# risc0/zeth

Measured on AMD Instinct MI355X. Metric: segments/sec, higher is better.
Workload: dtype u32

## Files before the change

zeth_amd/csrc/common.h:

```cpp
#pragma once
#include <hip/hip_runtime.h>

#include <atomic>
#include <cstdarg>
#include <cstdio>
#include <cstdlib>
#include <cstring>
#include <map>
#include <string>
#include <vector>

#include "../../include/zkhal.h"
#include "fp.h"
#include "noise.h"

namespace zkh {

inline const char* make_err(const char* fmt, ...) {
    char buf[512];
    va_list ap;
    va_start(ap, fmt);
    vsnprintf(buf, sizeof buf, fmt, ap);
    va_end(ap);
    return strdup(buf);
// ... 7 lines not shown
    do {                                 \
        const char* _err = (expr);       \
        if (_err) return _err;           \
    } while (0)
#define ZKH_REQUIRE(cond, ...)                         \
    do {                                               \
        if (!(cond)) return zkh::make_err(__VA_ARGS__); \
    } while (0)

constexpr int ZKH_P2_PTAB = 414;
constexpr int TW_BITS = 12;
constexpr int TW_SIZE = 1 << TW_BITS;
constexpr int TW_HI_BITS = 14;
constexpr int TW_HI_SIZE = 1 << TW_HI_BITS;
constexpr int MAX_LOG_N = TW_BITS + TW_HI_BITS;
constexpr int LDS_TW_LOG = 12;

struct DeviceTables {
    uint32_t* rc;
    uint32_t* diag;
    uint32_t* tw_fwd_lo; uint32_t* tw_fwd_hi;
    uint32_t* tw_rev_lo; uint32_t* tw_rev_hi;
    uint32_t* tile_fwd;  uint32_t* tile_rev;
    uint32_t* layer_fwd; uint32_t* layer_rev;
    uint32_t* layer_fwd_lazy;
    uint32_t* shift_lo;  uint32_t* shift_hi;
};

struct ProfAgg { uint64_t calls = 0; double ms = 0; double bytes = 0; };
struct ProfPending { std::string name; hipEvent_t a, b; double bytes; };

}

struct zkh_alloc_t {
    void* ptr;
    size_t bytes;
    std::atomic<int> refs;
    bool owned;
    zkh_ctx* ctx;
    zkh_alloc_t(void* p, size_t b, int r, bool o, zkh_ctx* c) : ptr(p), bytes(b), refs(r), owned(o), ctx(c) {}
};

struct zkh_buf {
    zkh_alloc_t* a;
    size_t off, len;
    std::atomic<int> refs;
    zkh_buf(zkh_alloc_t* al, size_t o, size_t l, int r) : a(al), off(o), len(l), refs(r) {}
    uint32_t* ptr() const { return (uint32_t*)a->ptr + off; }
// ... 68 lines not shown
```

zeth_amd/csrc/fp.h:

```cpp
#pragma once
#include <stdint.h>

#if defined(__HIPCC__)
#include <hip/hip_runtime.h>
#define ZKH_HD __host__ __device__ __forceinline__
#else
#define ZKH_HD inline
#endif

namespace zkh {

constexpr uint32_t P = 2013265921u;
constexpr uint32_t PINV = 0x88000001u;
constexpr uint32_t NEG_PINV = 0x77ffffffu;
constexpr uint32_t R1 = 268435454u;
constexpr uint32_t R2 = 1172168163u;
constexpr uint32_t INVALID = 0xffffffffu;

struct Fp {
    uint32_t v;
    ZKH_HD Fp() : v(0) {}
    ZKH_HD explicit constexpr Fp(uint32_t raw, int) : v(raw) {}
    static ZKH_HD Fp raw(uint32_t r) { return Fp(r, 0); }
    static ZKH_HD Fp one() { return Fp(R1, 0); }
// ... 33 lines not shown
    return d;
#else
    return (int64_t)((uint64_t)acc + (uint64_t)((int64_t)a * b));
#endif
}
ZKH_HD int64_t mad_i64_k(int32_t a, int32_t b_uniform, int64_t acc) {
#if defined(__HIP_DEVICE_COMPILE__)
    int64_t d; uint64_t carry;
    asm("v_mad_i64_i32 %0, %1, %2, %3, %4" : "=v"(d), "=s"(carry) : "v"(a), "s"(b_uniform), "v"(acc));
    return d;
#else
    return (int64_t)((uint64_t)acc + (uint64_t)((int64_t)a * b_uniform));
#endif
}
ZKH_HD int64_t mul_i64(int32_t a, int32_t b) {
#if defined(__HIP_DEVICE_COMPILE__)
    int64_t d; uint64_t carry;
    asm("v_mad_i64_i32 %0, %1, %2, %3, 0" : "=v"(d), "=s"(carry) : "v"(a), "v"(b));
    return d;
#else
    return (int64_t)a * b;
#endif
}
ZKH_HD int32_t smont_reduce(int64_t t) {
    const int32_t m = (int32_t)((uint32_t)t * NEG_PINV);
    return (int32_t)(mad_i64_k(m, (int32_t)P, t) >> 32);
}
ZKH_HD int32_t smont(int32_t a, int32_t b) {
    const int64_t t = (int64_t)a * b;
    const int32_t m = (int32_t)((uint32_t)t * NEG_PINV);
    const int64_t s = t + (int64_t)m * (int64_t)P;
    return (int32_t)(s >> 32);
}
ZKH_HD uint32_t canon(int32_t x) { const uint32_t u = (uint32_t)x, v = u + P; return v < u ? v : u; }
ZKH_HD int32_t center(uint32_t x) { return (int32_t)(x - (x > (P - 1) / 2 ? P : 0u)); }
ZKH_HD uint32_t mul_mod(uint32_t a, uint32_t b) { return mont_reduce((uint64_t)a * b); }

ZKH_HD Fp operator+(Fp a, Fp b) { return Fp::raw(add_mod(a.v, b.v)); }
ZKH_HD Fp operator-(Fp a, Fp b) { return Fp::raw(sub_mod(a.v, b.v)); }
ZKH_HD Fp operator*(Fp a, Fp b) { return Fp::raw(mul_mod(a.v, b.v)); }
ZKH_HD Fp operator-(Fp a) { return Fp::raw(a.v ? P - a.v : 0); }
ZKH_HD bool operator==(Fp a, Fp b) { return a.v == b.v; }
ZKH_HD Fp& operator+=(Fp& a, Fp b) { a = a + b; return a; }
ZKH_HD Fp& operator-=(Fp& a, Fp b) { a = a - b; return a; }
ZKH_HD Fp& operator*=(Fp& a, Fp b) { a = a * b; return a; }

ZKH_HD Fp fp_encode(uint32_t x) { return Fp::raw(mul_mod(R2, x % P)); }
ZKH_HD uint32_t fp_decode(Fp a) { return mul_mod(1u, a.v); }
ZKH_HD Fp fp_pow(Fp a, uint64_t e) {
    Fp r = Fp::one();
    while (e) { if (e & 1) r = r * a; a = a * a; e >>= 1; }
    return r;
}
ZKH_HD Fp fp_inv(Fp a) { return fp_pow(a, P - 2); }

constexpr uint32_t NBETA_CANON = P - 11;
// ... 79 lines not shown
```

zeth_amd/csrc/hal.hip:

```cpp
#include <algorithm>

#include "common.h"

#include <sys/random.h>
#include "poseidon2.h"
#include "ntt_lazy.h"
#include "../../include/zkh_poseidon2_consts.h"

using namespace zkh;

extern "C" void zkh_free_error(const char* e) { free((void*)e); }
#if ZKH_P2_CONSTS_ARE_PLACEHOLDER
extern "C" const char* zkh_version(void) { return "zkhal-mi355x 0.2.0 (gfx950; poseidon2_consts=placeholder)"; }
#elif ZKH_P2_CONSTS_ARE_DERIVED
extern "C" const char* zkh_version(void) { return "zkhal-mi355x 0.2.0 (gfx950; poseidon2_consts=derived)"; }
#else
extern "C" const char* zkh_version(void) { return "zkhal-mi355x 0.2.0 (gfx950; poseidon2_consts=upstream)"; }
#endif

namespace zkh {

const char* pool_alloc(zkh_ctx* c, size_t bytes, void** out) {
    bytes = (bytes + 255) & ~(size_t)255;
    if (bytes == 0) bytes = 256;
// ... 132 lines not shown
        delete c;
        return make_err("hipStreamCreateWithFlags: %s", hipGetErrorString(se));
    }
    if (const char* err = ctx_init_tables(c)) {
        zkh_ctx_destroy(c);
        return err;
    }
    *out = c;
    return nullptr;
}
static const char* ctx_init_tables(zkh_ctx* c) {
    Fp g = fp_encode(137);
    for (int k = 0; k <= 27; k++) {
        Fp w = fp_pow(g, 1ull << (27 - k));
        c->rou_fwd[k] = w.v;
        c->rou_rev[k] = fp_inv(w).v;
    }
    Fp wf = Fp::raw(c->rou_fwd[MAX_LOG_N]), wr = Fp::raw(c->rou_rev[MAX_LOG_N]);
    ZKH_TRY(upload(&c->tab.tw_fwd_lo, powers(wf, TW_SIZE)));
    ZKH_TRY(upload(&c->tab.tw_fwd_hi, powers(fp_pow(wf, TW_SIZE), TW_HI_SIZE)));
    ZKH_TRY(upload(&c->tab.tw_rev_lo, powers(wr, TW_SIZE)));
    ZKH_TRY(upload(&c->tab.tw_rev_hi, powers(fp_pow(wr, TW_SIZE), TW_HI_SIZE)));
    ZKH_TRY(upload(&c->tab.tile_fwd, powers(Fp::raw(c->rou_fwd[LDS_TW_LOG]), 1 << (LDS_TW_LOG - 1))));
    ZKH_TRY(upload(&c->tab.tile_rev, powers(Fp::raw(c->rou_rev[LDS_TW_LOG]), 1 << (LDS_TW_LOG - 1))));
    {
        std::vector<uint32_t> lf(1 << LDS_TW_LOG, R1), lr(1 << LDS_TW_LOG, R1);
        for (int j = 1; j <= LDS_TW_LOG; j++) {
            auto pf = powers(Fp::raw(c->rou_fwd[j]), (size_t)1 << (j - 1)), pr = powers(Fp::raw(c->rou_rev[j]), (size_t)1 << (j - 1));
            for (size_t e = 0; e < pf.size(); e++) { lf[((size_t)1 << (j - 1)) + e] = pf[e]; lr[((size_t)1 << (j - 1)) + e] = pr[e]; }
        }
        ZKH_TRY(upload(&c->tab.layer_fwd, lf));
        ZKH_TRY(upload(&c->tab.layer_rev, lr));
        static_assert(LAZY_TAB_LOG == LDS_TW_LOG, "the lazy table covers the per-layer tables");
        std::vector<uint32_t> lz(LAZY_TAB_WORDS);
        lazy_layer_table(lz.data(), lf.data());
        ZKH_TRY(upload(&c->tab.layer_fwd_lazy, lz));
    }
    Fp three = fp_encode(3);
    ZKH_TRY(upload(&c->tab.shift_lo, powers(three, TW_SIZE)));
    ZKH_TRY(upload(&c->tab.shift_hi, powers(fp_pow(three, TW_SIZE), TW_HI_SIZE)));
    ZKH_TRY(upload(&c->tab.rc, std::vector<uint32_t>(24 * 29)));
    ZKH_TRY(upload(&c->tab.diag, std::vector<uint32_t>(ZKH_P2_PTAB)));
    ZKH_TRY(zkh_poseidon2_set_constants(c, ZKH_P2_ROUND_CONSTANTS, ZKH_P2_M_INT_DIAG));
    ZKH_TRY(ntt_device_init(c));
    ZKH_HIP(hipMalloc((void**)&c->d_fail, 8));
    ZKH_HIP(hipMemsetAsync(c->d_fail, 0, 8, c->stream));
    ZKH_HIP(hipHostMalloc((void**)&c->h_fail, 8, hipHostMallocDefault));
    c->h_fail[0] = c->h_fail[1] = 0;
    return nullptr;
}
extern "C" const char* zkh_ctx_trim(zkh_ctx* c) {
    bind_thread(c);
    ZKH_HIP(hipStreamSynchronize(c->stream));
    for (auto& kv : c->pool) (void)hipFree(kv.second);
    c->pool.clear(); c->pool_bytes = 0;
    return nullptr;
}
extern "C" void zkh_ctx_memory(const zkh_ctx* c, size_t* live, size_t* cached, size_t* peak) {
    if (live) *live = c->live_bytes;
    if (cached) *cached = c->pool_bytes;
    if (peak) *peak = c->peak_bytes;
}
extern "C" void zkh_ctx_destroy(zkh_ctx* c) {
    if (!c) return;
    (void)hipSetDevice(c->device);
    (void)hipStreamSynchronize(c->stream);
    for (auto& kv : c->pool) (void)hipFree(kv.second);
    uint32_t* t[] = {c->tab.rc, c->tab.diag, c->tab.tw_fwd_lo, c->tab.tw_fwd_hi, c->tab.tw_rev_lo, c->tab.tw_rev_hi,
                     c->tab.tile_fwd, c->tab.tile_rev, c->tab.shift_lo, c->tab.shift_hi, c->tab.layer_fwd, c->tab.layer_rev, c->tab.layer_fwd_lazy};
    for (auto p : t) (void)hipFree(p);
    for (auto& p : c->pending) { (void)hipEventDestroy(p.a); (void)hipEventDestroy(p.b); }
    for (auto ev : c->event_pool) (void)hipEventDestroy(ev);
    if (c->pinned) (void)hipHostFree(c->pinned);
    if (c->d_fail) (void)hipFree(c->d_fail);
    if (c->h_fail) (void)hipHostFree(c->h_fail);
    for (auto& kv : c->host_blocks) (void)hipHostFree(kv.first);
    (void)hipStreamDestroy(c->stream);
    delete c;
}
static const char* check_device_fail(zkh_ctx* c) {
    if (!c->fail_armed) return nullptr;
    c->fail_armed = false;
    const uint32_t code = c->h_fail[0], detail = c->h_fail[1];
    if (!code) return nullptr;
    (void)hipMemsetAsync(c->d_fail, 0, 8, c->stream);
    switch (code) {
    case 1: return make_err("combos_prepare_regs: register %u has size 0 or more than `cycles` words (found on the device; the call's combos are unchanged)", detail);
    case 2: return make_err("combos_prepare_regs: register %u names a combo beyond combo_count (found on the device; the call's combos are unchanged)", detail);
    case 3: return make_err("combos_prepare_regs: the register sizes add up to %u U coefficients (+ %d of the check polynomial), more than coeff_u holds (found on the device; the call's combos are unchanged)", detail, ZKH_CHECK_SIZE);
    default: return make_err("a kernel reported failure code %u (%u)", code, detail);
    }
}
// ... 373 lines not shown
```

zeth_amd/csrc/ntt.hip:

```cpp
#include "common.h"
#include "ntt_lazy.h"

using namespace zkh;

namespace {

constexpr int NTT_THREADS = 256;

struct PassParams {
    const uint32_t* in;
    uint32_t* out;
    size_t in_col_stride;
    size_t out_col_stride;
    uint32_t log_n;
    uint32_t L, R;
    uint32_t log_t;
    uint32_t expand_bits;
    uint32_t first_layer;
    uint32_t twiddle;
    uint32_t scale;
    uint32_t zk_shift;
    const uint32_t* tile_tw;
    const uint32_t* layer_tw;
    const uint32_t* tw_lo;
// ... 188 lines not shown
    __syncthreads();
    for (uint32_t e = threadIdx.x; e < H * H; e += blockDim.x) {
        const uint32_t hi2 = e >> BR_H, lo2 = e & (H - 1);
        const uint32_t shi = __brev(lo2) >> (32 - BR_H), slo = __brev(hi2) >> (32 - BR_H);
        const uint32_t src = (shi << BR_H) | slo;
        col[((size_t)hi2 << (log_n - BR_H)) | ((size_t)rmid << BR_H) | lo2] = ta[src];
        if (rmid != mid) col[((size_t)hi2 << (log_n - BR_H)) | ((size_t)mid << BR_H) | lo2] = tb[src];
    }
}
__global__ void k_bit_reverse_small(uint32_t* io, uint32_t log_n, size_t count) {
    size_t g = (size_t)blockIdx.x * blockDim.x + threadIdx.x;
    size_t n = (size_t)1 << log_n;
    if (g >= n * count) return;
    uint32_t i = (uint32_t)(g & (n - 1));
    uint32_t r = log_n ? __brev(i) >> (32 - log_n) : 0;
    if (i < r) {
        uint32_t* col = io + (g - i);
        uint32_t x = col[i], y = col[r];
        col[i] = y; col[r] = x;
    }
}


template <int LOGR, bool INVERSE, bool BASE0, int J_LO, bool LAZY = false>
__device__ __forceinline__ void radix_layers(uint32_t (&v)[1 << LOGR], const uint32_t* __restrict__ ltab,
                                             const uint32_t base_low, const int first_b) {
    constexpr int N = 1 << LOGR;
    if (!INVERSE && LAZY) {
        lazy_layers<LOGR, BASE0, J_LO>(v, ltab, base_low, first_b);
    } else if (INVERSE) {
#pragma unroll
        for (int b = LOGR - 1; b >= 0; b--) {
            const uint32_t* tw = ltab + (1u << (J_LO + b - 1));
#pragma unroll
            for (int kk = 0; kk < (1 << b); kk++) {
                const bool unit = BASE0 && kk == 0;
                const uint32_t w = unit ? 0u : tw[base_low + ((uint32_t)kk << (J_LO - 1))];
#pragma unroll
                for (int hi = 0; hi < (N >> (b + 1)); hi++) {
                    const int k = (hi << (b + 1)) | kk;
                    const uint32_t x = v[k], y = v[k + (1 << b)];
                    v[k] = add_mod(x, y);
                    v[k + (1 << b)] = unit ? sub_mod(x, y) : mul_mod(x - y + P, w);
                }
            }
        }
    } else {
#pragma unroll
        for (int b = 0; b < LOGR; b++) {
            if (b < first_b) continue;
            const uint32_t* tw = ltab + (1u << (J_LO + b - 1));
#pragma unroll
            for (int kk = 0; kk < (1 << b); kk++) {
                const bool unit = BASE0 && kk == 0;
                const uint32_t w = unit ? 0u : tw[base_low + ((uint32_t)kk << (J_LO - 1))];
#pragma unroll
                for (int hi = 0; hi < (N >> (b + 1)); hi++) {
                    const int k = (hi << (b + 1)) | kk;
                    const uint32_t x = v[k], y = unit ? v[k + (1 << b)] : mul_mod(v[k + (1 << b)], w);
                    v[k] = add_mod(x, y);
                    v[k + (1 << b)] = sub_mod(x, y);
                }
            }
        }
    }
}

template <bool INVERSE, bool LAZY = false>
__global__ __launch_bounds__(256) void k_ntt_low12(PassParams p) {
    __shared__ __attribute__((aligned(16))) uint32_t lds[4096];
    const uint32_t tid = threadIdx.x;
    const uint32_t tile = xcd_remap(blockIdx.x, p.tiles_per_col);
    const size_t base = (size_t)tile << 12;
    const uint32_t* in = p.in + (size_t)blockIdx.y * p.in_col_stride;
    uint32_t* out = p.out + (size_t)blockIdx.y * p.out_col_stride;
    const uint32_t* __restrict__ ltab = p.layer_tw;
    const uint32_t hi = tid >> 4, low = tid & 15;
    uint32_t v[16];
    if (INVERSE) {
#pragma unroll
        for (int k = 0; k < 16; k++) v[k] = in[base + k * 256 + tid];
        radix_layers<4, true, false, 9>(v, ltab, tid, 0);
#pragma unroll
        for (int k = 0; k < 16; k++) lds[k * 256 + tid] = v[k];
        __syncthreads();
#pragma unroll
        for (int k = 0; k < 16; k++) v[k] = lds[hi * 256 + k * 16 + low];
        radix_layers<4, true, false, 5>(v, ltab, low, 0);
#pragma unroll
        for (int k = 0; k < 16; k++) lds[hi * 256 + k * 16 + low] = v[k];
        __syncthreads();
#pragma unroll
        for (int q = 0; q < 4; q++) {
            const uint4 w = ((const uint4*)lds)[tid * 4 + q];
            v[4 * q] = w.x; v[4 * q + 1] = w.y; v[4 * q + 2] = w.z; v[4 * q + 3] = w.w;
        }
        radix_layers<4, true, true, 1>(v, ltab, 0, 0);
        const size_t pos0 = base + (size_t)tid * 16;
        if (p.zk_shift) {
            const uint32_t ex = __brev((uint32_t)pos0) >> (32 - p.log_n);
            const uint32_t b = mul_mod(p.sh_lo[ex & (TW_SIZE - 1)], p.sh_hi[ex >> TW_BITS]);
#pragma unroll
            for (int k = 0; k < 16; k++) v[k] = mul_mod(mul_mod(v[k], b), p.shift16[k]);
        } else if (p.scale) {
#pragma unroll
            for (int k = 0; k < 16; k++) v[k] = mul_mod(v[k], p.scale);
        }
#pragma unroll
        for (int q = 0; q < 4; q++) ((uint4*)(out + pos0))[q] = make_uint4(v[4 * q], v[4 * q + 1], v[4 * q + 2], v[4 * q + 3]);
    } else {
        const size_t pos0 = base + (size_t)tid * 16;
        if (p.expand_bits == 0) {
#pragma unroll
            for (int q = 0; q < 4; q++) {
                const uint4 w = ((const uint4*)(in + pos0))[q];
                v[4 * q] = w.x; v[4 * q + 1] = w.y; v[4 * q + 2] = w.z; v[4 * q + 3] = w.w;
            }
        } else if (p.expand_bits == 2) {
            const uint4 w = *(const uint4*)(in + (pos0 >> 2));
            v[0] = v[1] = v[2] = v[3] = w.x; v[4] = v[5] = v[6] = v[7] = w.y;
            v[8] = v[9] = v[10] = v[11] = w.z; v[12] = v[13] = v[14] = v[15] = w.w;
        } else {
#pragma unroll
            for (int k = 0; k < 16; k++) v[k] = in[(pos0 + k) >> p.expand_bits];
        }
        radix_layers<4, false, true, 1, LAZY>(v, ltab, 0, (int)p.expand_bits);
#pragma unroll
        for (int q = 0; q < 4; q++) ((uint4*)lds)[tid * 4 + q] = make_uint4(v[4 * q], v[4 * q + 1], v[4 * q + 2], v[4 * q + 3]);
        __syncthreads();
#pragma unroll
        for (int k = 0; k < 16; k++) v[k] = lds[hi * 256 + k * 16 + low];
        radix_layers<4, false, false, 5, LAZY>(v, ltab, low, 0);
#pragma unroll
        for (int k = 0; k < 16; k++) lds[hi * 256 + k * 16 + low] = v[k];
        __syncthreads();
#pragma unroll
        for (int k = 0; k < 16; k++) v[k] = lds[k * 256 + tid];
        radix_layers<4, false, false, 9, LAZY>(v, ltab, tid, 0);
#pragma unroll
        for (int k = 0; k < 16; k++) out[base + k * 256 + tid] = v[k];
    }
}

template <int RH, bool INVERSE, bool LAZY = false>
__global__ __launch_bounds__(1 << RH) void k_ntt_high(PassParams p) {
    constexpr int LT = 4;
    constexpr uint32_t TW = 1u << LT;
    extern __shared__ __attribute__((aligned(16))) uint32_t lds[];
    const uint32_t tid = threadIdx.x, t = tid & (TW - 1), g = tid >> LT;
    const uint32_t tile_id = xcd_remap(blockIdx.x, p.tiles_per_col), col = blockIdx.y;
    const uint32_t lt_bits = p.L - LT;
    const uint32_t a = tile_id >> lt_bits, lt = tile_id & ((1u << lt_bits) - 1);
    const size_t base = ((size_t)a << (p.L + RH)) + ((size_t)lt << LT);
    const uint32_t lcol = (lt << LT) + t;
    const uint32_t tw_shift = MAX_LOG_N - (p.L + RH);
    const char* in = (const char*)(p.in + (size_t)col * p.in_col_stride + base);
    char* out = (char*)(p.out + (size_t)col * p.out_col_stride + base);
    const uint32_t tb = t * 4u;
#define TILE_IN(row) (*(const uint32_t*)(in + ((((uint32_t)(row)) << (p.L + 2)) + tb)))
#define TILE_OUT(row) (*(uint32_t*)(out + ((((uint32_t)(row)) << (p.L + 2)) + tb)))
    const uint32_t* __restrict__ ltab = p.layer_tw;
    auto tmul = [](uint32_t x, uint32_t y) -> uint32_t {
        return (LAZY && !INVERSE) ? (uint32_t)smont((int32_t)x, (int32_t)y) : mul_mod(x, y);
    };
    auto root = [&](uint32_t e) -> uint32_t {
        const uint32_t ex = e << tw_shift;
        return tmul(p.tw_lo[ex & (TW_SIZE - 1)], p.tw_hi[ex >> TW_BITS]);
    };
    uint32_t tw[16];
    if (RH == 10) {
        uint32_t w0 = root(lcol * (__brev(g) >> 26));
        if (LAZY) w0 = tmul(w0, p.lazy_comp);
        const uint32_t u1 = root(lcol * 64u), v1 = root(lcol * 256u);
        const uint32_t u2 = tmul(u1, u1), u3 = tmul(u2, u1), v2 = tmul(v1, v1), v3 = tmul(v2, v1);
        const uint32_t wi[4] = {w0, tmul(w0, u2), tmul(w0, u1), tmul(w0, u3)};
#pragma unroll
        for (int i = 0; i < 4; i++) {
            tw[4 * i] = wi[i]; tw[4 * i + 1] = tmul(wi[i], v2); tw[4 * i + 2] = tmul(wi[i], v1); tw[4 * i + 3] = tmul(wi[i], v3);
        }
    } else {
        uint32_t w0 = root(lcol * (__brev(g) >> 28));
        if (LAZY) w0 = tmul(w0, p.lazy_comp);
        const uint32_t q1 = root(lcol * 16u);
        uint32_t qp[16];
        qp[0] = w0;
#pragma unroll
        for (int e = 1; e < 16; e++) qp[e] = tmul(qp[e - 1], q1);
#pragma unroll
        for (int k = 0; k < 16; k++) tw[k] = qp[__builtin_bitreverse8((unsigned char)k) >> 4];
    }
    uint32_t v[16];
    if (RH == 10) {
        const uint32_t hi = g >> 2, low = g & 3;
        if (INVERSE) {
#pragma unroll
            for (int k = 0; k < 16; k++) v[k] = TILE_IN(k * 64 + g);
            radix_layers<4, true, false, 7>(v, ltab, g, 0);
#pragma unroll
            for (int k = 0; k < 16; k++) lds[(k * 64 + g) * TW + t] = v[k];
            __syncthreads();
#pragma unroll
            for (int k = 0; k < 16; k++) v[k] = lds[(hi * 64 + k * 4 + low) * TW + t];
            radix_layers<4, true, false, 3>(v, ltab, low, 0);
#pragma unroll
            for (int k = 0; k < 16; k++) lds[(hi * 64 + k * 4 + low) * TW + t] = v[k];
            __syncthreads();
#pragma unroll
            for (int i = 0; i < 4; i++) {
                uint32_t u[4];
                const uint32_t m0 = (g * 4 + i) * 4;
#pragma unroll
                for (int k = 0; k < 4; k++) u[k] = lds[(m0 + k) * TW + t];
                radix_layers<2, true, true, 1>(u, ltab, 0, 0);
#pragma unroll
                for (int k = 0; k < 4; k++) {
                    uint32_t x = mul_mod(u[k], tw[4 * i + k]);
                    if (p.scale) x = mul_mod(x, p.scale);
                    TILE_OUT(m0 + k) = x;
                }
            }
        } else {
#pragma unroll
            for (int i = 0; i < 4; i++) {
                uint32_t u[4];
                const uint32_t m0 = (g * 4 + i) * 4;
#pragma unroll
                for (int k = 0; k < 4; k++) {
                    const uint32_t x = TILE_IN(m0 + k);
                    u[k] = LAZY ? (uint32_t)smont((int32_t)x, (int32_t)tw[4 * i + k]) : mul_mod(x, tw[4 * i + k]);
                }
                radix_layers<2, false, true, 1, LAZY>(u, ltab, 0, 0);
#pragma unroll
                for (int k = 0; k < 4; k++) lds[(m0 + k) * TW + t] = u[k];
            }
            __syncthreads();
#pragma unroll
            for (int k = 0; k < 16; k++) v[k] = lds[(hi * 64 + k * 4 + low) * TW + t];
            radix_layers<4, false, false, 3, LAZY>(v, ltab, low, 0);
#pragma unroll
            for (int k = 0; k < 16; k++) lds[(hi * 64 + k * 4 + low) * TW + t] = v[k];
            __syncthreads();
#pragma unroll
            for (int k = 0; k < 16; k++) v[k] = lds[(k * 64 + g) * TW + t];
            radix_layers<4, false, false, 7, LAZY>(v, ltab, g, 0);
#pragma unroll
            for (int k = 0; k < 16; k++) TILE_OUT(k * 64 + g) = LAZY ? canon((int32_t)v[k]) : v[k];
        }
    } else {
        if (INVERSE) {
#pragma unroll
            for (int k = 0; k < 16; k++) v[k] = TILE_IN(k * 16 + g);
            radix_layers<4, true, false, 5>(v, ltab, g, 0);
#pragma unroll
            for (int k = 0; k < 16; k++) lds[(k * 16 + g) * TW + t] = v[k];
            __syncthreads();
#pragma unroll
            for (int k = 0; k < 16; k++) v[k] = lds[(g * 16 + k) * TW + t];
            radix_layers<4, true, true, 1>(v, ltab, 0, 0);
#pragma unroll
            for (int k = 0; k < 16; k++) {
                uint32_t x = mul_mod(v[k], tw[k]);
                if (p.scale) x = mul_mod(x, p.scale);
                TILE_OUT(g * 16 + k) = x;
            }
        } else {
#pragma unroll
            for (int k = 0; k < 16; k++) {
                const uint32_t x = TILE_IN(g * 16 + k);
                v[k] = LAZY ? (uint32_t)smont((int32_t)x, (int32_t)tw[k]) : mul_mod(x, tw[k]);
            }
            radix_layers<4, false, true, 1, LAZY>(v, ltab, 0, 0);
#pragma unroll
            for (int k = 0; k < 16; k++) lds[(g * 16 + k) * TW + t] = v[k];
            __syncthreads();
#pragma unroll
            for (int k = 0; k < 16; k++) v[k] = lds[(k * 16 + g) * TW + t];
            radix_layers<4, false, false, 5, LAZY>(v, ltab, g, 0);
#pragma unroll
            for (int k = 0; k < 16; k++) TILE_OUT(k * 16 + g) = LAZY ? canon((int32_t)v[k]) : v[k];
        }
    }
}
#undef TILE_IN
#undef TILE_OUT

struct Pass { uint32_t L, R; };
std::vector<Pass> plan_passes(uint32_t log_n) {
    std::vector<Pass> v;
    if (log_n <= 12) { v.push_back({0, log_n}); return v; }
    if (log_n < 18) {
        const uint32_t low = (log_n + 1) / 2;
        v.push_back({0, low});
        v.push_back({low, log_n - low});
        return v;
    }
    const uint32_t rem = log_n - 12;
    v.push_back({0, 12});
    if (rem == 8 || rem == 10 || rem <= 7) v.push_back({12, rem});
    else if (rem == 9) { v.push_back({12, 8}); v.push_back({20, 1}); }
    else if (rem == 11 || rem == 12) { v.push_back({12, 8}); v.push_back({20, rem - 8}); }
// ... 11 lines not shown
    const size_t npass = passes.size();
    const bool lazy = !inverse && npass == 2 && passes[0].R == 12 && (passes[1].R == 8 || passes[1].R == 10) && expand_bits <= 4;
    const uint32_t lazy_reds = lazy ? lazy_reductions(4, expand_bits) + 2 * lazy_reductions(4, 0) + lazy_reductions(passes[1].R, 0) : 0;
    const uint32_t lazy_comp = lazy ? fp_pow(Fp::raw(R2), lazy_reds).v : 0;
    for (size_t pi = 0; pi < npass; pi++) {
        const Pass ps = inverse ? passes[npass - 1 - pi] : passes[pi];
        PassParams p{};
        const bool first = pi == 0, last = pi + 1 == npass;
        p.in = first ? in : out;
        p.in_col_stride = first ? in_col_stride : out_col_stride;
        p.out = out; p.out_col_stride = out_col_stride;
        p.log_n = log_n; p.L = ps.L; p.R = ps.R;
        const bool reg_high = ps.L >= 4 && (ps.R == 8 || ps.R == 10);
        p.log_t = ps.L == 0 ? 0 : (ps.L < 4 ? ps.L : 4);
        if (ps.L != 0 && !reg_high && ps.R < 12) p.log_t = std::max<uint32_t>(p.log_t, std::min<uint32_t>(ps.L, 12 - ps.R));
        while (p.R + p.log_t > 14 && p.log_t > 0) p.log_t--;
        p.expand_bits = (!inverse && first) ? expand_bits : 0;
        p.first_layer = (!inverse && first) ? expand_bits + 1 : 1;
        p.twiddle = ps.L != 0;
        p.scale = (inverse && last) ? ninv.v : 0;
        p.zk_shift = (inverse && last && zk) ? 1 : 0;
        p.lazy = lazy; p.lazy_comp = lazy_comp;
        p.tile_tw = inverse ? c->tab.tile_rev : c->tab.tile_fwd;
        p.layer_tw = inverse ? c->tab.layer_rev : (lazy ? c->tab.layer_fwd_lazy : c->tab.layer_fwd);
        p.tw_lo = inverse ? c->tab.tw_rev_lo : c->tab.tw_fwd_lo;
        p.tw_hi = inverse ? c->tab.tw_rev_hi : c->tab.tw_fwd_hi;
        p.sh_lo = c->tab.shift_lo; p.sh_hi = c->tab.shift_hi;
        if (p.zk_shift && log_n >= 4) {
            const Fp three = fp_encode(3);
            for (uint32_t k = 0; k < 16; k++)
                p.shift16[k] = (ninv * fp_pow(three, (uint64_t)(bitrev32(k) >> 28) << (log_n - 4))).v;
        }
        p.tiles_per_col = (uint32_t)(n >> (p.R + p.log_t));
        const size_t lds = ((size_t)4 << (p.R + p.log_t));
        dim3 grid(p.tiles_per_col, (unsigned)count);
        const double alg_bytes = pi == 0 ? 4.0 * count * (double)(((size_t)1 << log_n) >> expand_bits) + 4.0 * count * (double)n : 0.0;
        const bool scale_here = p.scale != 0;
        const bool k_low = ps.L == 0 && ps.R == 12 && p.expand_bits <= 4;
        const bool k_h10 = !k_low && ps.L >= 4 && p.log_t == 4 && ps.R == 10 && !(scale_here && p.zk_shift);
        const bool k_h8 = !k_low && !k_h10 && ps.L >= 4 && p.log_t == 4 && ps.R == 8 && !(scale_here && p.zk_shift);
        const bool k_top = !k_low && !k_h10 && !k_h8 && ps.L >= 12 && ps.L + ps.R == log_n && ps.R >= 1 && ps.R <= 4 && p.twiddle &&
                           p.expand_bits == 0 && p.first_layer == 1 && !scale_here && !p.zk_shift;
        const std::string pname = std::string(name) + (k_low ? ":k_ntt_low12" : k_h10 ? ":k_ntt_high10" : k_h8 ? ":k_ntt_high8" : k_top ? ":k_ntt_top" : ":k_ntt_pass");
        ProfScope prof(c, pname.c_str(), alg_bytes);
        if (ps.L == 0 && ps.R == 12 && p.expand_bits <= 4) {
            if (inverse) k_ntt_low12<true><<<grid, 256, 0, c->stream>>>(p);
            else if (lazy) k_ntt_low12<false, true><<<grid, 256, 0, c->stream>>>(p);
            else k_ntt_low12<false><<<grid, 256, 0, c->stream>>>(p);
        } else if (ps.L >= 4 && p.log_t == 4 && ps.R == 10 && !(scale_here && p.zk_shift)) {
            if (inverse) k_ntt_high<10, true><<<grid, 1024, lds, c->stream>>>(p);
            else if (lazy) k_ntt_high<10, false, true><<<grid, 1024, lds, c->stream>>>(p);
            else k_ntt_high<10, false><<<grid, 1024, lds, c->stream>>>(p);
        } else if (ps.L >= 4 && p.log_t == 4 && ps.R == 8 && !(scale_here && p.zk_shift)) {
            if (inverse) k_ntt_high<8, true><<<grid, 256, lds, c->stream>>>(p);
            else if (lazy) k_ntt_high<8, false, true><<<grid, 256, lds, c->stream>>>(p);
            else k_ntt_high<8, false><<<grid, 256, lds, c->stream>>>(p);
        } else if (k_top) {
            const dim3 tg((unsigned)(((size_t)1 << ps.L) >> 10), (unsigned)count);
            switch (ps.R * 2 + (inverse ? 1 : 0)) {
            case 2: k_ntt_top<1, false><<<tg, 256, 0, c->stream>>>(p); break;
            case 3: k_ntt_top<1, true><<<tg, 256, 0, c->stream>>>(p); break;
            case 4: k_ntt_top<2, false><<<tg, 256, 0, c->stream>>>(p); break;
            case 5: k_ntt_top<2, true><<<tg, 256, 0, c->stream>>>(p); break;
            case 6: k_ntt_top<3, false><<<tg, 256, 0, c->stream>>>(p); break;
            case 7: k_ntt_top<3, true><<<tg, 256, 0, c->stream>>>(p); break;
            case 8: k_ntt_top<4, false><<<tg, 256, 0, c->stream>>>(p); break;
            default: k_ntt_top<4, true><<<tg, 256, 0, c->stream>>>(p); break;
            }
        } else if (inverse) k_ntt_pass<true><<<grid, NTT_THREADS, lds, c->stream>>>(p);
        else k_ntt_pass<false><<<grid, NTT_THREADS, lds, c->stream>>>(p);
        ZKH_TRY(last_launch_error(name));
    }
    return nullptr;
}

}

const char* zkh::ntt_device_init(zkh_ctx* c) {
    bind_thread(c);
    ZKH_HIP(hipFuncSetAttribute((const void*)k_ntt_high<10, true>, hipFuncAttributeMaxDynamicSharedMemorySize, 65536));
    ZKH_HIP(hipFuncSetAttribute((const void*)k_ntt_high<10, false>, hipFuncAttributeMaxDynamicSharedMemorySize, 65536));
    ZKH_HIP(hipFuncSetAttribute((const void*)k_ntt_high<10, false, true>, hipFuncAttributeMaxDynamicSharedMemorySize, 65536));
    return nullptr;
}

static const char* interpolate_impl(zkh_ctx* c, zkh_buf* io, size_t count, bool zk, const char* name) {
    ZKH_REQUIRE(count && io->len % count == 0, "%s: size %zu not a multiple of count %zu", name, io->len, count);
    const size_t n = io->len / count;
    const uint32_t log_n = log2_ceil(n);
    ZKH_REQUIRE(((size_t)1 << log_n) == n, "%s: column length %zu is not a power of two", name, n);
    return run_transform(c, true, io->ptr(), n, io->ptr(), n, log_n, count, 0, zk, name);
}
extern "C" const char* zkh_batch_interpolate_ntt(zkh_ctx* c, zkh_buf* io, size_t count) {
    return interpolate_impl(c, io, count, false, "batch_interpolate_ntt");
}
extern "C" const char* zkh_batch_interpolate_ntt_zk_shift(zkh_ctx* c, zkh_buf* io, size_t count) {
    return interpolate_impl(c, io, count, true, "batch_interpolate_ntt_zk_shift");
}
extern "C" const char* zkh_batch_interpolate_ntt_from(zkh_ctx* c, zkh_buf* out, const zkh_buf* in, size_t count, int zk_shift) {
    ZKH_REQUIRE(count && in->len % count == 0 && out->len == in->len, "batch_interpolate_ntt_from: shape mismatch");
    const size_t n = in->len / count;
    const uint32_t log_n = log2_ceil(n);
    ZKH_REQUIRE(((size_t)1 << log_n) == n, "batch_interpolate_ntt_from: column length %zu is not a power of two", n);
// ... 40 lines not shown
```

zeth_amd/csrc/ntt_lazy.h:

```cpp
#pragma once
#include "fp.h"

#ifndef ZKH_LAZY_SUM
#define ZKH_LAZY_SUM(t) ((void)0)
#endif

namespace zkh {

constexpr int LAZY_TAB_LOG = 12;
constexpr uint32_t LAZY_TAB_MONT = 1u << LAZY_TAB_LOG;
constexpr uint32_t LAZY_TAB_WORDS = 2u << LAZY_TAB_LOG;

inline void lazy_layer_table(uint32_t* out, const uint32_t* layer_fwd) {
    for (uint32_t i = 0; i < LAZY_TAB_MONT; i++) {
        out[i] = (uint32_t)center(mont_reduce((uint64_t)layer_fwd[i]));
        out[LAZY_TAB_MONT + i] = (uint32_t)center(layer_fwd[i]);
    }
}

template <bool UNIFORM>
ZKH_HD int64_t lazy_mad(int32_t a, int32_t w, int64_t acc) {
    if constexpr (UNIFORM) return mad_i64_k(a, w, acc);
    else return mad_i64(a, w, acc);
}
ZKH_HD int32_t lazy_reduce(int64_t t) {
    ZKH_LAZY_SUM(t);
    return smont_reduce(t);
}

template <bool UNIFORM>
ZKH_HD void lazy_single(uint32_t& v0, uint32_t& v1, int32_t w) {
    const int64_t x = (int64_t)(int32_t)v0;
    const int32_t y = (int32_t)v1, nw = -w;
    v0 = (uint32_t)lazy_reduce(lazy_mad<UNIFORM>(y, w, x));
    v1 = (uint32_t)lazy_reduce(lazy_mad<UNIFORM>(y, nw, x));
}

template <bool UNIFORM>
ZKH_HD void lazy_pair(uint32_t& v0, uint32_t& v1, uint32_t& v2, uint32_t& v3, int32_t wa, int32_t wb0, int32_t wb1) {
// ... 30 lines not shown
                const int32_t wb0 = (BASE0 && kk == 0) ? (int32_t)R1 : (int32_t)twb[e];
                const int32_t wb1 = (int32_t)twb[e + ((1u << b) << (J_LO - 1))];
#pragma unroll
                for (int hi = 0; hi < (N >> (b + 2)); hi++) {
                    const int k = (hi << (b + 2)) | kk;
                    lazy_pair<BASE0>(v[k], v[k + (1 << b)], v[k + (2 << b)], v[k + (3 << b)], wa, wb0, wb1);
                }
            }
        } else if (b + 1 >= first_b) {
            const uint32_t* tw1 = ltab + (1u << (J_LO + b));
#pragma unroll
            for (int kk = 0; kk < (2 << b); kk++) {
                const int32_t w = (BASE0 && kk == 0) ? 1 : (int32_t)tw1[base_low + ((uint32_t)kk << (J_LO - 1))];
#pragma unroll
                for (int hi = 0; hi < (N >> (b + 2)); hi++) {
                    const int k = (hi << (b + 2)) | kk;
                    lazy_single<BASE0>(v[k], v[k + (2 << b)], w);
                }
            }
        }
    }
}

}
```

Measured before the change: 44.35.

## Port inverse NTT register-radix kernels to lazy signed Montgomery radix-4 butterflies

Replaces the inverse radix-2 Gentleman-Sande layers in the low12 and high kernels with lazy signed radix-4 butterflies backed by a new bit-reversed inverse twiddle table. This removes per-layer canonical reductions and halves the number of reduction rounds. The Montgomery compensation factor is folded into the final scale or shift multipliers, and a signed-output variant skips canonicalisation when the next pass is the lazy low kernel. In exchange it adds complexity in the scale bookkeeping and depends on signed intermediate bounds holding across passes.

```diff
diff --git a/zeth_amd/csrc/common.h b/zeth_amd/csrc/common.h
--- a/zeth_amd/csrc/common.h
+++ b/zeth_amd/csrc/common.h
@@ -53,8 +53,9 @@
     uint32_t* tw_fwd_lo; uint32_t* tw_fwd_hi;
     uint32_t* tw_rev_lo; uint32_t* tw_rev_hi;
     uint32_t* tile_fwd;  uint32_t* tile_rev;
-    uint32_t* layer_fwd; uint32_t* layer_rev;
+    uint32_t* layer_fwd;
     uint32_t* layer_fwd_lazy;
+    uint32_t* layer_rev_lazy;
     uint32_t* shift_lo;  uint32_t* shift_hi;
 };
 
diff --git a/zeth_amd/csrc/fp.h b/zeth_amd/csrc/fp.h
--- a/zeth_amd/csrc/fp.h
+++ b/zeth_amd/csrc/fp.h
@@ -79,6 +79,15 @@
     return (int64_t)a * b;
 #endif
 }
+ZKH_HD int64_t mul_i64_k(int32_t a, int32_t b_uniform) {
+#if defined(__HIP_DEVICE_COMPILE__)
+    int64_t d; uint64_t carry;
+    asm("v_mad_i64_i32 %0, %1, %2, %3, 0" : "=v"(d), "=s"(carry) : "v"(a), "s"(b_uniform));
+    return d;
+#else
+    return (int64_t)a * b_uniform;
+#endif
+}
 ZKH_HD int32_t smont_reduce(int64_t t) {
     const int32_t m = (int32_t)((uint32_t)t * NEG_PINV);
     return (int32_t)(mad_i64_k(m, (int32_t)P, t) >> 32);
@@ -89,6 +98,8 @@
     const int64_t s = t + (int64_t)m * (int64_t)P;
     return (int32_t)(s >> 32);
 }
+ZKH_HD int32_t smont_v(int32_t a, int32_t b) { return smont_reduce(mul_i64(a, b)); }
+ZKH_HD int32_t smont_k(int32_t a, int32_t b_uniform) { return smont_reduce(mul_i64_k(a, b_uniform)); }
 ZKH_HD uint32_t canon(int32_t x) { const uint32_t u = (uint32_t)x, v = u + P; return v < u ? v : u; }
 ZKH_HD int32_t center(uint32_t x) { return (int32_t)(x - (x > (P - 1) / 2 ? P : 0u)); }
 ZKH_HD uint32_t mul_mod(uint32_t a, uint32_t b) { return mont_reduce((uint64_t)a * b); }
diff --git a/zeth_amd/csrc/hal.hip b/zeth_amd/csrc/hal.hip
--- a/zeth_amd/csrc/hal.hip
+++ b/zeth_amd/csrc/hal.hip
@@ -178,19 +178,21 @@
     ZKH_TRY(upload(&c->tab.tw_rev_lo, powers(wr, TW_SIZE)));
     ZKH_TRY(upload(&c->tab.tw_rev_hi, powers(fp_pow(wr, TW_SIZE), TW_HI_SIZE)));
     ZKH_TRY(upload(&c->tab.tile_fwd, powers(Fp::raw(c->rou_fwd[LDS_TW_LOG]), 1 << (LDS_TW_LOG - 1))));
-    ZKH_TRY(upload(&c->tab.tile_rev, powers(Fp::raw(c->rou_rev[LDS_TW_LOG]), 1 << (LDS_TW_LOG - 1))));
+    const std::vector<uint32_t> tile_rev = powers(Fp::raw(c->rou_rev[LDS_TW_LOG]), 1 << (LDS_TW_LOG - 1));
+    ZKH_TRY(upload(&c->tab.tile_rev, tile_rev));
     {
-        std::vector<uint32_t> lf(1 << LDS_TW_LOG, R1), lr(1 << LDS_TW_LOG, R1);
+        std::vector<uint32_t> lf(1 << LDS_TW_LOG, R1);
         for (int j = 1; j <= LDS_TW_LOG; j++) {
-            auto pf = powers(Fp::raw(c->rou_fwd[j]), (size_t)1 << (j - 1)), pr = powers(Fp::raw(c->rou_rev[j]), (size_t)1 << (j - 1));
-            for (size_t e = 0; e < pf.size(); e++) { lf[((size_t)1 << (j - 1)) + e] = pf[e]; lr[((size_t)1 << (j - 1)) + e] = pr[e]; }
+            auto pf = powers(Fp::raw(c->rou_fwd[j]), (size_t)1 << (j - 1));
+            for (size_t e = 0; e < pf.size(); e++) lf[((size_t)1 << (j - 1)) + e] = pf[e];
         }
         ZKH_TRY(upload(&c->tab.layer_fwd, lf));
-        ZKH_TRY(upload(&c->tab.layer_rev, lr));
-        static_assert(LAZY_TAB_LOG == LDS_TW_LOG, "the lazy table covers the per-layer tables");
-        std::vector<uint32_t> lz(LAZY_TAB_WORDS);
+        static_assert(LAZY_TAB_LOG == LDS_TW_LOG, "the lazy tables cover the per-layer tables");
+        std::vector<uint32_t> lz(LAZY_TAB_WORDS), li(LAZY_INV_WORDS);
         lazy_layer_table(lz.data(), lf.data());
         ZKH_TRY(upload(&c->tab.layer_fwd_lazy, lz));
+        lazy_inv_table(li.data(), tile_rev.data());
+        ZKH_TRY(upload(&c->tab.layer_rev_lazy, li));
     }
     Fp three = fp_encode(3);
     ZKH_TRY(upload(&c->tab.shift_lo, powers(three, TW_SIZE)));
@@ -223,7 +225,7 @@
     (void)hipStreamSynchronize(c->stream);
     for (auto& kv : c->pool) (void)hipFree(kv.second);
     uint32_t* t[] = {c->tab.rc, c->tab.diag, c->tab.tw_fwd_lo, c->tab.tw_fwd_hi, c->tab.tw_rev_lo, c->tab.tw_rev_hi,
-                     c->tab.tile_fwd, c->tab.tile_rev, c->tab.shift_lo, c->tab.shift_hi, c->tab.layer_fwd, c->tab.layer_rev, c->tab.layer_fwd_lazy};
+                     c->tab.tile_fwd, c->tab.tile_rev, c->tab.shift_lo, c->tab.shift_hi, c->tab.layer_fwd, c->tab.layer_fwd_lazy, c->tab.layer_rev_lazy};
     for (auto p : t) (void)hipFree(p);
     for (auto& p : c->pending) { (void)hipEventDestroy(p.a); (void)hipEventDestroy(p.b); }
     for (auto ev : c->event_pool) (void)hipEventDestroy(ev);
diff --git a/zeth_amd/csrc/ntt.hip b/zeth_amd/csrc/ntt.hip
--- a/zeth_amd/csrc/ntt.hip
+++ b/zeth_amd/csrc/ntt.hip
@@ -234,29 +234,12 @@
 }
 
 
-template <int LOGR, bool INVERSE, bool BASE0, int J_LO, bool LAZY = false>
+template <int LOGR, bool BASE0, int J_LO, bool LAZY = false>
 __device__ __forceinline__ void radix_layers(uint32_t (&v)[1 << LOGR], const uint32_t* __restrict__ ltab,
                                              const uint32_t base_low, const int first_b) {
     constexpr int N = 1 << LOGR;
-    if (!INVERSE && LAZY) {
+    if (LAZY) {
         lazy_layers<LOGR, BASE0, J_LO>(v, ltab, base_low, first_b);
-    } else if (INVERSE) {
-#pragma unroll
-        for (int b = LOGR - 1; b >= 0; b--) {
-            const uint32_t* tw = ltab + (1u << (J_LO + b - 1));
-#pragma unroll
-            for (int kk = 0; kk < (1 << b); kk++) {
-                const bool unit = BASE0 && kk == 0;
-                const uint32_t w = unit ? 0u : tw[base_low + ((uint32_t)kk << (J_LO - 1))];
-#pragma unroll
-                for (int hi = 0; hi < (N >> (b + 1)); hi++) {
-                    const int k = (hi << (b + 1)) | kk;
-                    const uint32_t x = v[k], y = v[k + (1 << b)];
-                    v[k] = add_mod(x, y);
-                    v[k + (1 << b)] = unit ? sub_mod(x, y) : mul_mod(x - y + P, w);
-                }
-            }
-        }
     } else {
 #pragma unroll
         for (int b = 0; b < LOGR; b++) {
@@ -280,6 +263,7 @@
 
 template <bool INVERSE, bool LAZY = false>
 __global__ __launch_bounds__(256) void k_ntt_low12(PassParams p) {
+    static_assert(!INVERSE || LAZY, "the inverse register-radix kernels are lazy");
     __shared__ __attribute__((aligned(16))) uint32_t lds[4096];
     const uint32_t tid = threadIdx.x;
     const uint32_t tile = xcd_remap(blockIdx.x, p.tiles_per_col);
@@ -292,13 +276,13 @@
     if (INVERSE) {
 #pragma unroll
         for (int k = 0; k < 16; k++) v[k] = in[base + k * 256 + tid];
-        radix_layers<4, true, false, 9>(v, ltab, tid, 0);
+        lazy_layers_inv<4, true>(v, ltab, 0);
 #pragma unroll
         for (int k = 0; k < 16; k++) lds[k * 256 + tid] = v[k];
         __syncthreads();
 #pragma unroll
         for (int k = 0; k < 16; k++) v[k] = lds[hi * 256 + k * 16 + low];
-        radix_layers<4, true, false, 5>(v, ltab, low, 0);
+        lazy_layers_inv<4, false>(v, ltab, hi);
 #pragma unroll
         for (int k = 0; k < 16; k++) lds[hi * 256 + k * 16 + low] = v[k];
         __syncthreads();
@@ -307,16 +291,16 @@
             const uint4 w = ((const uint4*)lds)[tid * 4 + q];
             v[4 * q] = w.x; v[4 * q + 1] = w.y; v[4 * q + 2] = w.z; v[4 * q + 3] = w.w;
         }
-        radix_layers<4, true, true, 1>(v, ltab, 0, 0);
+        lazy_layers_inv<4, false>(v, ltab, tid);
         const size_t pos0 = base + (size_t)tid * 16;
         if (p.zk_shift) {
             const uint32_t ex = __brev((uint32_t)pos0) >> (32 - p.log_n);
-            const uint32_t b = mul_mod(p.sh_lo[ex & (TW_SIZE - 1)], p.sh_hi[ex >> TW_BITS]);
-#pragma unroll
-            for (int k = 0; k < 16; k++) v[k] = mul_mod(mul_mod(v[k], b), p.shift16[k]);
-        } else if (p.scale) {
-#pragma unroll
-            for (int k = 0; k < 16; k++) v[k] = mul_mod(v[k], p.scale);
+            const int32_t b = smont((int32_t)p.sh_lo[ex & (TW_SIZE - 1)], (int32_t)p.sh_hi[ex >> TW_BITS]);
+#pragma unroll
+            for (int k = 0; k < 16; k++) v[k] = canon(smont_k(smont_v((int32_t)v[k], b), (int32_t)p.shift16[k]));
+        } else {
+#pragma unroll
+            for (int k = 0; k < 16; k++) v[k] = canon(smont_k((int32_t)v[k], (int32_t)p.scale));
         }
 #pragma unroll
         for (int q = 0; q < 4; q++) ((uint4*)(out + pos0))[q] = make_uint4(v[4 * q], v[4 * q + 1], v[4 * q + 2], v[4 * q + 3]);
@@ -336,26 +320,27 @@
 #pragma unroll
             for (int k = 0; k < 16; k++) v[k] = in[(pos0 + k) >> p.expand_bits];
         }
-        radix_layers<4, false, true, 1, LAZY>(v, ltab, 0, (int)p.expand_bits);
+        radix_layers<4, true, 1, LAZY>(v, ltab, 0, (int)p.expand_bits);
 #pragma unroll
         for (int q = 0; q < 4; q++) ((uint4*)lds)[tid * 4 + q] = make_uint4(v[4 * q], v[4 * q + 1], v[4 * q + 2], v[4 * q + 3]);
         __syncthreads();
 #pragma unroll
         for (int k = 0; k < 16; k++) v[k] = lds[hi * 256 + k * 16 + low];
-        radix_layers<4, false, false, 5, LAZY>(v, ltab, low, 0);
+        radix_layers<4, false, 5, LAZY>(v, ltab, low, 0);
 #pragma unroll
         for (int k = 0; k < 16; k++) lds[hi * 256 + k * 16 + low] = v[k];
         __syncthreads();
 #pragma unroll
         for (int k = 0; k < 16; k++) v[k] = lds[k * 256 + tid];
-        radix_layers<4, false, false, 9, LAZY>(v, ltab, tid, 0);
+        radix_layers<4, false, 9, LAZY>(v, ltab, tid, 0);
 #pragma unroll
         for (int k = 0; k < 16; k++) out[base + k * 256 + tid] = v[k];
     }
 }
 
-template <int RH, bool INVERSE, bool LAZY = false>
+template <int RH, bool INVERSE, bool LAZY = false, bool SIGNED_OUT = false>
 __global__ __launch_bounds__(1 << RH) void k_ntt_high(PassParams p) {
+    static_assert(!INVERSE || LAZY, "the inverse register-radix kernels are lazy");
     constexpr int LT = 4;
     constexpr uint32_t TW = 1u << LT;
     extern __shared__ __attribute__((aligned(16))) uint32_t lds[];
@@ -373,7 +358,11 @@
 #define TILE_OUT(row) (*(uint32_t*)(out + ((((uint32_t)(row)) << (p.L + 2)) + tb)))
     const uint32_t* __restrict__ ltab = p.layer_tw;
     auto tmul = [](uint32_t x, uint32_t y) -> uint32_t {
-        return (LAZY && !INVERSE) ? (uint32_t)smont((int32_t)x, (int32_t)y) : mul_mod(x, y);
+        return LAZY ? (uint32_t)smont((int32_t)x, (int32_t)y) : mul_mod(x, y);
+    };
+    auto inv_out = [&](uint32_t x, uint32_t w) -> uint32_t {
+        const int32_t y = smont((int32_t)x, (int32_t)w);
+        return SIGNED_OUT ? (uint32_t)y : canon(y);
     };
     auto root = [&](uint32_t e) -> uint32_t {
         const uint32_t ex = e << tw_shift;
@@ -407,13 +396,13 @@
         if (INVERSE) {
 #pragma unroll
             for (int k = 0; k < 16; k++) v[k] = TILE_IN(k * 64 + g);
-            radix_layers<4, true, false, 7>(v, ltab, g, 0);
+            lazy_layers_inv<4, true>(v, ltab, 0);
 #pragma unroll
             for (int k = 0; k < 16; k++) lds[(k * 64 + g) * TW + t] = v[k];
             __syncthreads();
 #pragma unroll
             for (int k = 0; k < 16; k++) v[k] = lds[(hi * 64 + k * 4 + low) * TW + t];
-            radix_layers<4, true, false, 3>(v, ltab, low, 0);
+            lazy_layers_inv<4, false>(v, ltab, hi);
 #pragma unroll
             for (int k = 0; k < 16; k++) lds[(hi * 64 + k * 4 + low) * TW + t] = v[k];
             __syncthreads();
@@ -423,13 +412,9 @@
                 const uint32_t m0 = (g * 4 + i) * 4;
 #pragma unroll
                 for (int k = 0; k < 4; k++) u[k] = lds[(m0 + k) * TW + t];
-                radix_layers<2, true, true, 1>(u, ltab, 0, 0);
-#pragma unroll
-                for (int k = 0; k < 4; k++) {
-                    uint32_t x = mul_mod(u[k], tw[4 * i + k]);
-                    if (p.scale) x = mul_mod(x, p.scale);
-                    TILE_OUT(m0 + k) = x;
-                }
+                lazy_layers_inv<2, false>(u, ltab, g * 4 + i);
+#pragma unroll
+                for (int k = 0; k < 4; k++) TILE_OUT(m0 + k) = inv_out(u[k], tw[4 * i + k]);
             }
         } else {
 #pragma unroll
@@ -441,20 +426,20 @@
                     const uint32_t x = TILE_IN(m0 + k);
                     u[k] = LAZY ? (uint32_t)smont((int32_t)x, (int32_t)tw[4 * i + k]) : mul_mod(x, tw[4 * i + k]);
                 }
-                radix_layers<2, false, true, 1, LAZY>(u, ltab, 0, 0);
+                radix_layers<2, true, 1, LAZY>(u, ltab, 0, 0);
 #pragma unroll
                 for (int k = 0; k < 4; k++) lds[(m0 + k) * TW + t] = u[k];
             }
             __syncthreads();
 #pragma unroll
             for (int k = 0; k < 16; k++) v[k] = lds[(hi * 64 + k * 4 + low) * TW + t];
-            radix_layers<4, false, false, 3, LAZY>(v, ltab, low, 0);
+            radix_layers<4, false, 3, LAZY>(v, ltab, low, 0);
 #pragma unroll
             for (int k = 0; k < 16; k++) lds[(hi * 64 + k * 4 + low) * TW + t] = v[k];
             __syncthreads();
 #pragma unroll
             for (int k = 0; k < 16; k++) v[k] = lds[(k * 64 + g) * TW + t];
-            radix_layers<4, false, false, 7, LAZY>(v, ltab, g, 0);
+            radix_layers<4, false, 7, LAZY>(v, ltab, g, 0);
 #pragma unroll
             for (int k = 0; k < 16; k++) TILE_OUT(k * 64 + g) = LAZY ? canon((int32_t)v[k]) : v[k];
         }
@@ -462,32 +447,28 @@
         if (INVERSE) {
 #pragma unroll
             for (int k = 0; k < 16; k++) v[k] = TILE_IN(k * 16 + g);
-            radix_layers<4, true, false, 5>(v, ltab, g, 0);
+            lazy_layers_inv<4, true>(v, ltab, 0);
 #pragma unroll
             for (int k = 0; k < 16; k++) lds[(k * 16 + g) * TW + t] = v[k];
             __syncthreads();
 #pragma unroll
             for (int k = 0; k < 16; k++) v[k] = lds[(g * 16 + k) * TW + t];
-            radix_layers<4, true, true, 1>(v, ltab, 0, 0);
-#pragma unroll
-            for (int k = 0; k < 16; k++) {
-                uint32_t x = mul_mod(v[k], tw[k]);
-                if (p.scale) x = mul_mod(x, p.scale);
-                TILE_OUT(g * 16 + k) = x;
-            }
+            lazy_layers_inv<4, false>(v, ltab, g);
+#pragma unroll
+            for (int k = 0; k < 16; k++) TILE_OUT(g * 16 + k) = inv_out(v[k], tw[k]);
         } else {
 #pragma unroll
             for (int k = 0; k < 16; k++) {
                 const uint32_t x = TILE_IN(g * 16 + k);
                 v[k] = LAZY ? (uint32_t)smont((int32_t)x, (int32_t)tw[k]) : mul_mod(x, tw[k]);
             }
-            radix_layers<4, false, true, 1, LAZY>(v, ltab, 0, 0);
+            radix_layers<4, true, 1, LAZY>(v, ltab, 0, 0);
 #pragma unroll
             for (int k = 0; k < 16; k++) lds[(g * 16 + k) * TW + t] = v[k];
             __syncthreads();
 #pragma unroll
             for (int k = 0; k < 16; k++) v[k] = lds[(k * 16 + g) * TW + t];
-            radix_layers<4, false, false, 5, LAZY>(v, ltab, g, 0);
+            radix_layers<4, false, 5, LAZY>(v, ltab, g, 0);
 #pragma unroll
             for (int k = 0; k < 16; k++) TILE_OUT(k * 16 + g) = LAZY ? canon((int32_t)v[k]) : v[k];
         }
@@ -545,20 +526,29 @@
         p.zk_shift = (inverse && last && zk) ? 1 : 0;
         p.lazy = lazy; p.lazy_comp = lazy_comp;
         p.tile_tw = inverse ? c->tab.tile_rev : c->tab.tile_fwd;
-        p.layer_tw = inverse ? c->tab.layer_rev : (lazy ? c->tab.layer_fwd_lazy : c->tab.layer_fwd);
+        p.layer_tw = inverse ? c->tab.layer_rev_lazy : (lazy ? c->tab.layer_fwd_lazy : c->tab.layer_fwd);
         p.tw_lo = inverse ? c->tab.tw_rev_lo : c->tab.tw_fwd_lo;
         p.tw_hi = inverse ? c->tab.tw_rev_hi : c->tab.tw_fwd_hi;
         p.sh_lo = c->tab.shift_lo; p.sh_hi = c->tab.shift_hi;
+        const bool inv_low = inverse && ps.L == 0 && ps.R == 12, inv_high = inverse && reg_high && p.log_t == 4 && !(last && zk);
+        Fp inv_scale = ninv;
+        if (inv_low || inv_high) {
+            const Fp comp = fp_pow(Fp::raw(R2), ps.R / 2);
+            inv_scale = ninv * comp;
+            if (inv_low) p.scale = inv_scale.v;
+            else p.lazy_comp = (last ? inv_scale : comp).v;
+        }
         if (p.zk_shift && log_n >= 4) {
             const Fp three = fp_encode(3);
             for (uint32_t k = 0; k < 16; k++)
-                p.shift16[k] = (ninv * fp_pow(three, (uint64_t)(bitrev32(k) >> 28) << (log_n - 4))).v;
+                p.shift16[k] = (inv_scale * fp_pow(three, (uint64_t)(bitrev32(k) >> 28) << (log_n - 4))).v;
         }
         p.tiles_per_col = (uint32_t)(n >> (p.R + p.log_t));
         const size_t lds = ((size_t)4 << (p.R + p.log_t));
         dim3 grid(p.tiles_per_col, (unsigned)count);
         const double alg_bytes = pi == 0 ? 4.0 * count * (double)(((size_t)1 << log_n) >> expand_bits) + 4.0 * count * (double)n : 0.0;
         const bool scale_here = p.scale != 0;
+        const bool signed_out = inverse && !last && passes[npass - 2 - pi].L == 0 && passes[npass - 2 - pi].R == 12;
         const bool k_low = ps.L == 0 && ps.R == 12 && p.expand_bits <= 4;
         const bool k_h10 = !k_low && ps.L >= 4 && p.log_t == 4 && ps.R == 10 && !(scale_here && p.zk_shift);
         const bool k_h8 = !k_low && !k_h10 && ps.L >= 4 && p.log_t == 4 && ps.R == 8 && !(scale_here && p.zk_shift);
@@ -567,15 +557,17 @@
         const std::string pname = std::string(name) + (k_low ? ":k_ntt_low12" : k_h10 ? ":k_ntt_high10" : k_h8 ? ":k_ntt_high8" : k_top ? ":k_ntt_top" : ":k_ntt_pass");
         ProfScope prof(c, pname.c_str(), alg_bytes);
         if (ps.L == 0 && ps.R == 12 && p.expand_bits <= 4) {
-            if (inverse) k_ntt_low12<true><<<grid, 256, 0, c->stream>>>(p);
+            if (inverse) k_ntt_low12<true, true><<<grid, 256, 0, c->stream>>>(p);
             else if (lazy) k_ntt_low12<false, true><<<grid, 256, 0, c->stream>>>(p);
             else k_ntt_low12<false><<<grid, 256, 0, c->stream>>>(p);
         } else if (ps.L >= 4 && p.log_t == 4 && ps.R == 10 && !(scale_here && p.zk_shift)) {
-            if (inverse) k_ntt_high<10, true><<<grid, 1024, lds, c->stream>>>(p);
+            if (inverse && signed_out) k_ntt_high<10, true, true, true><<<grid, 1024, lds, c->stream>>>(p);
+            else if (inverse) k_ntt_high<10, true, true><<<grid, 1024, lds, c->stream>>>(p);
             else if (lazy) k_ntt_high<10, false, true><<<grid, 1024, lds, c->stream>>>(p);
             else k_ntt_high<10, false><<<grid, 1024, lds, c->stream>>>(p);
         } else if (ps.L >= 4 && p.log_t == 4 && ps.R == 8 && !(scale_here && p.zk_shift)) {
-            if (inverse) k_ntt_high<8, true><<<grid, 256, lds, c->stream>>>(p);
+            if (inverse && signed_out) k_ntt_high<8, true, true, true><<<grid, 256, lds, c->stream>>>(p);
+            else if (inverse) k_ntt_high<8, true, true><<<grid, 256, lds, c->stream>>>(p);
             else if (lazy) k_ntt_high<8, false, true><<<grid, 256, lds, c->stream>>>(p);
             else k_ntt_high<8, false><<<grid, 256, lds, c->stream>>>(p);
         } else if (k_top) {
@@ -601,7 +593,8 @@
 
 const char* zkh::ntt_device_init(zkh_ctx* c) {
     bind_thread(c);
-    ZKH_HIP(hipFuncSetAttribute((const void*)k_ntt_high<10, true>, hipFuncAttributeMaxDynamicSharedMemorySize, 65536));
+    ZKH_HIP(hipFuncSetAttribute((const void*)k_ntt_high<10, true, true>, hipFuncAttributeMaxDynamicSharedMemorySize, 65536));
+    ZKH_HIP(hipFuncSetAttribute((const void*)k_ntt_high<10, true, true, true>, hipFuncAttributeMaxDynamicSharedMemorySize, 65536));
     ZKH_HIP(hipFuncSetAttribute((const void*)k_ntt_high<10, false>, hipFuncAttributeMaxDynamicSharedMemorySize, 65536));
     ZKH_HIP(hipFuncSetAttribute((const void*)k_ntt_high<10, false, true>, hipFuncAttributeMaxDynamicSharedMemorySize, 65536));
     return nullptr;
diff --git a/zeth_amd/csrc/ntt_lazy.h b/zeth_amd/csrc/ntt_lazy.h
--- a/zeth_amd/csrc/ntt_lazy.h
+++ b/zeth_amd/csrc/ntt_lazy.h
@@ -15,6 +15,16 @@
     for (uint32_t i = 0; i < LAZY_TAB_MONT; i++) {
         out[i] = (uint32_t)center(mont_reduce((uint64_t)layer_fwd[i]));
         out[LAZY_TAB_MONT + i] = (uint32_t)center(layer_fwd[i]);
+    }
+}
+
+constexpr uint32_t LAZY_INV_MONT = 1u << (LAZY_TAB_LOG - 1);
+constexpr uint32_t LAZY_INV_WORDS = 2u << (LAZY_TAB_LOG - 1);
+inline void lazy_inv_table(uint32_t* out, const uint32_t* tile_rev) {
+    for (uint32_t h = 0; h < LAZY_INV_MONT; h++) {
+        const uint32_t w = tile_rev[bitrev32(h) >> (33 - LAZY_TAB_LOG)];
+        out[h] = (uint32_t)center(mont_reduce((uint64_t)w));
+        out[LAZY_INV_MONT + h] = (uint32_t)center(w);
     }
 }
 
@@ -91,4 +101,25 @@
     }
 }
 
+template <int LOGR, bool TOP>
+ZKH_HD void lazy_layers_inv(uint32_t (&v)[1 << LOGR], const uint32_t* __restrict__ itab, const uint32_t H) {
+    static_assert(LOGR % 2 == 0, "lazy rounds hold an even number of layers");
+#pragma unroll
+    for (int b = LOGR - 2; b >= 0; b -= 2) {
+        const uint32_t* twa = itab + (H << (LOGR - 2 - b));
+        const uint32_t* twb = itab + LAZY_INV_MONT + (H << (LOGR - 1 - b));
+#pragma unroll
+        for (int q = 0; q < (1 << (LOGR - 2 - b)); q++) {
+            const int32_t wa = (TOP && q == 0) ? 1 : (int32_t)twa[q];
+            const int32_t wb0 = (TOP && q == 0) ? (int32_t)R1 : (int32_t)twb[2 * q];
+            const int32_t wb1 = (int32_t)twb[2 * q + 1];
+#pragma unroll
+            for (int kk = 0; kk < (1 << b); kk++) {
+                const int k = (q << (b + 2)) | kk;
+                lazy_pair<TOP>(v[k], v[k + (2 << b)], v[k + (1 << b)], v[k + (3 << b)], wa, wb0, wb1);
+            }
+        }
+    }
 }
+
+}
```

Result: no change. 44.33 (-0.0%).
